# Gorilla-Lab-SCUT/frustum-convnet

Measured on AMD Instinct MI355X. Metric: frustums/sec (train fwd+bwd) KITTI-car B=32 N=1024, higher is better.
Workload: dtype f32 (fp32 operands split into two 16-bit parts, 3 MFMAs per product, fp32 accumulate); 1 GPU; cfgs/det_sample.yaml KITTI-car, batch=32/GPU, Npoint=1024, L=(280,140,70,35), train fwd+bwd+Adam; global_batch=32, parallelism=dp1

## Files before the change

frustum_convnet_amd/csrc/fcn_tuning.h:

```cpp
#pragma once

#ifndef FCN_EXP
#define FCN_EXP 0
#endif
#define MM_ENC_W ((FCN_EXP & 1) ? MM_F32 : MM)
#define MM_ENC_A ((FCN_EXP & 2) ? MM_F32 : MM)

#ifndef FCN_X
#define FCN_X 0
#endif

#ifndef FCN_XB
#define FCN_XB 0
#endif

#ifndef FCN_XF
#define FCN_XF 0
#endif
#ifndef FCN_XG
#define FCN_XG 0
#endif

#ifdef FCN_TUNING_PNF
#ifdef FCN_PROBE
// ... 18 lines not shown
    unsigned int n = 0;
    if (hipMemcpyFromSymbol(&n, HIP_SYMBOL(g_pnf_probe_n), sizeof(n)) != hipSuccess) return -1;
    if ((int)n > max_records) n = max_records;
    if (n > PNF_MAX) n = PNF_MAX;
    if (n && hipMemcpyFromSymbol(host_out, HIP_SYMBOL(g_pnf_probe), (size_t)n * 8 * sizeof(unsigned long long)) != hipSuccess) return -1;
    if (reset) { unsigned int z = 0; hipMemcpyToSymbol(HIP_SYMBOL(g_pnf_probe_n), &z, sizeof(z)); }
    return (int)n;
}
#else
#define PNF_DECL
#define PNF_ADD(i)
#define PNF_FLUSH(tag)
#endif
#endif

#ifdef FCN_TUNING_PNP
#ifdef FCN_PROBE
#define PNP_MAX 32768
__device__ unsigned long long g_pn_probe[PNP_MAX * 8];
__device__ unsigned int g_pn_probe_n;
#define PNP_DECL unsigned long long pa_[6] = {0, 0, 0, 0, 0, 0}; unsigned long long pt_ = clock64(), pt0_ = pt_
#define PNP_ADD(i) do { const unsigned long long n_ = clock64(); pa_[i] += n_ - pt_; pt_ = n_; } while (0)
#define PNP_FLUSH(tag)                                                                                   \
    do {                                                                                                 \
        if (threadIdx.x == 0) {                                                                          \
            const unsigned int s_ = atomicAdd(&g_pn_probe_n, 1u);                                        \
            if (s_ < PNP_MAX) {                                                                          \
                g_pn_probe[s_ * 8] = (unsigned long long)(tag);                                          \
                g_pn_probe[s_ * 8 + 1] = clock64() - pt0_;                                               \
                for (int q_ = 0; q_ < 6; ++q_) g_pn_probe[s_ * 8 + 2 + q_] = pa_[q_];                    \
            }                                                                                            \
        }                                                                                                \
    } while (0)
extern "C" int fcn_pn_probe_read(unsigned long long *host_out, int max_records, int reset)
{
    unsigned int n = 0;
    if (hipMemcpyFromSymbol(&n, HIP_SYMBOL(g_pn_probe_n), sizeof(n)) != hipSuccess) return -1;
    if ((int)n > max_records) n = max_records;
    if (n > PNP_MAX) n = PNP_MAX;
    if (n && hipMemcpyFromSymbol(host_out, HIP_SYMBOL(g_pn_probe), (size_t)n * 8 * sizeof(unsigned long long)) != hipSuccess) return -1;
    if (reset) { unsigned int z = 0; hipMemcpyToSymbol(HIP_SYMBOL(g_pn_probe_n), &z, sizeof(z)); }
    return (int)n;
}
#else
#define PNP_DECL
#define PNP_ADD(i)
#define PNP_FLUSH(tag)
#endif
#endif

#ifdef FCN_TUNING_FCN
#ifdef FCN_PROBE
#define FCN_PROBE_MAX 65536
__device__ unsigned long long g_fcn_probe[FCN_PROBE_MAX * 8];
__device__ unsigned int g_fcn_probe_n;
#define PROBE_DECL unsigned long long pb_[8]; int pbn_ = 0
#define PROBE_STAMP() do { if (pbn_ < 7) pb_[pbn_++] = wall_clock64(); } while (0)
#define PROBE_FLUSH(tag)                                                                                 \
    do {                                                                                                 \
        if (threadIdx.x == 0) {                                                                          \
            const unsigned int s_ = atomicAdd(&g_fcn_probe_n, 1u);                                       \
            if (s_ < FCN_PROBE_MAX) {                                                                    \
                g_fcn_probe[s_ * 8] = (unsigned long long)(tag);                                         \
                for (int q_ = 0; q_ < 7; ++q_) g_fcn_probe[s_ * 8 + 1 + q_] = q_ < pbn_ ? pb_[q_] : 0ull; \
            }                                                                                            \
        }                                                                                                \
    } while (0)
extern "C" int fcn_probe_read(unsigned long long *host_out, int max_records, int reset)
{
    unsigned int n = 0;
    if (hipMemcpyFromSymbol(&n, HIP_SYMBOL(g_fcn_probe_n), sizeof(n)) != hipSuccess) return -1;
    if ((int)n > max_records) n = max_records;
    if (n > FCN_PROBE_MAX) n = FCN_PROBE_MAX;
    if (n && hipMemcpyFromSymbol(host_out, HIP_SYMBOL(g_fcn_probe), (size_t)n * 8 * sizeof(unsigned long long)) != hipSuccess) return -1;
    if (reset) { unsigned int z = 0; hipMemcpyToSymbol(HIP_SYMBOL(g_fcn_probe_n), &z, sizeof(z)); }
    return (int)n;
}
#else
#define PROBE_DECL
#define PROBE_STAMP()
#define PROBE_FLUSH(tag)
#endif
#if defined(FCN_PROBE) && FCN_PROBE >= 3
#define BPROBE_DECL unsigned long long pb_[8]; int pbn_ = 0
#define BPROBE_STAMP() do { if (pbn_ < 7) pb_[pbn_++] = wall_clock64(); } while (0)
#define BPROBE_FLUSH(tag) PROBE_FLUSH(tag)
#else
#define BPROBE_DECL
#define BPROBE_STAMP()
#define BPROBE_FLUSH(tag)
#endif
#endif

#ifndef FCN_POOL_FUSED
#define FCN_POOL_FUSED 1
#endif
```

frustum_convnet_amd/csrc/gemm_tile.h:

```cpp
#pragma once
#include "fcn_common.h"
#include "fcn_tuning.h"

typedef float v4f __attribute__((ext_vector_type(4)));
typedef int v4i __attribute__((ext_vector_type(4)));
typedef const v4f __attribute__((address_space(1))) *gv4fp;
typedef const v4i __attribute__((address_space(1))) *gv4ip;
__device__ __forceinline__ v4f ldg4(const float *p) { return *(gv4fp)p; }
__device__ __forceinline__ v4i ldg4i(const int *p) { return *(gv4ip)p; }
__device__ __forceinline__ void sts4(float *p, v4f v) { *(v4f *)p = v; }
__device__ __forceinline__ v4f zero4() { v4f z = {0.f, 0.f, 0.f, 0.f}; return z; }


#define GT 256

static inline bool fcn_pn_key_pool(const fcn_pn_desc *d, const fcn_pn_ws *ws, int C3)
{
    return FCN_POOL_FUSED && d->nlc && ws->pkey && ws->ewin && C3 % 2 == 0 && C3 <= 2 * GT && (2 * GT) % C3 == 0;
}
#define KC 32

#define MM_F32 0
#define MM_F16X3 1
#define MM_BF16X3 2
// ... 236 lines not shown
    } else {
#pragma unroll
        for (int q = 0; q < 4; ++q) {
            float h, l;
            enc2<MM>(x[2 * q], x[2 * q + 1], h, l);
            hi[q] = __builtin_bit_cast(uint32_t, h);
            lo[q] = __builtin_bit_cast(uint32_t, l);
        }
    }
}

typedef float v2f_kb __attribute__((ext_vector_type(2)));
template <int MM, int LDR>
__device__ __forceinline__ void kb_store4(u32x4 *img, int r, int kq, float x0, float x1, float x2, float x3)
{
    const int kb = kq >> 1, half = kq & 1;
    if constexpr (MM == MM_F32) {
        const v4f v = {x0, x1, x2, x3};
        *(v4f *)(img + (half * 4 + kb) * LDR + r) = v;
    } else {
        float h0, l0, h1, l1;
        enc2<MM>(x0, x1, h0, l0);
        enc2<MM>(x2, x3, h1, l1);
        const v2f_kb h = {h0, h1}, l = {l0, l1};
        *(v2f_kb *)((float *)(img + kb * LDR + r) + 2 * half) = h;
        if constexpr (!mm_x1<MM>) *(v2f_kb *)((float *)(img + (4 + kb) * LDR + r) + 2 * half) = l;
    }
}

typedef const u32x4 __attribute__((address_space(1))) *gu4p;
__device__ __forceinline__ u32x4 ldgu4(const u32x4 *p) { return *(gu4p)p; }

template <int MM, int MT, int NT, int LDRA, int LDRB>
__device__ __forceinline__ void mma_chunk_kb(const u32x4 *A, const u32x4 *B, int arow0, int bcol0, f32x16 (&acc)[MT][NT])
{
    const int lane = threadIdx.x & 63;
    const int l31 = lane & 31, lh = lane >> 5;
    if constexpr (MM == MM_F32) {
        const float *Af = (const float *)A, *Bf = (const float *)B;
#pragma unroll
        for (int kk = 0; kk < KC; kk += 2) {
            const int k = kk + lh, kb = k >> 3, j = k & 7;
            float a[MT], b[NT];
#pragma unroll
            for (int i = 0; i < MT; ++i) a[i] = Af[(((j >> 2) * 4 + kb) * LDRA + arow0 + i * 32 + l31) * 4 + (j & 3)];
#pragma unroll
            for (int jn = 0; jn < NT; ++jn) b[jn] = Bf[(((j >> 2) * 4 + kb) * LDRB + bcol0 + jn * 32 + l31) * 4 + (j & 3)];
#pragma unroll
            for (int i = 0; i < MT; ++i)
#pragma unroll
                for (int jn = 0; jn < NT; ++jn)
                    acc[i][jn] = __builtin_amdgcn_mfma_f32_32x32x2f32(a[i], b[jn], acc[i][jn], 0, 0, 0);
        }
    } else {
        constexpr bool X3 = !mm_x1<MM>;
        const u32x4 *ap = A + lh * LDRA + arow0 + l31;
        const u32x4 *bp = B + lh * LDRB + bcol0 + l31;
#pragma unroll
        for (int ks = 0; ks < 2; ++ks) {
            u32x4 ah[MT], al[MT], bh[NT], bl[NT];
#pragma unroll
            for (int i = 0; i < MT; ++i) {
                ah[i] = ap[2 * ks * LDRA + i * 32];
                if constexpr (X3) al[i] = ap[(4 + 2 * ks) * LDRA + i * 32];
            }
#pragma unroll
            for (int j = 0; j < NT; ++j) {
                bh[j] = bp[2 * ks * LDRB + j * 32];
                if constexpr (X3) bl[j] = bp[(4 + 2 * ks) * LDRB + j * 32];
            }
            if constexpr (X3) {
#pragma unroll
                for (int i = 0; i < MT; ++i)
#pragma unroll
                    for (int j = 0; j < NT; ++j) acc[i][j] = mfma16<MM>(ah[i], bl[j], acc[i][j]);
#pragma unroll
                for (int i = 0; i < MT; ++i)
#pragma unroll
                    for (int j = 0; j < NT; ++j) acc[i][j] = mfma16<MM>(al[i], bh[j], acc[i][j]);
            }
#pragma unroll
            for (int i = 0; i < MT; ++i)
#pragma unroll
                for (int j = 0; j < NT; ++j) acc[i][j] = mfma16<MM>(ah[i], bh[j], acc[i][j]);
        }
    }
}

#define EP_LD 32
#define EP_FLOATS (32 * EP_LD)
__device__ __forceinline__ void ep_put(float *patch, const f32x16 &acc, int l31, int lh)
{
#pragma unroll
    for (int reg = 0; reg < 16; ++reg) patch[acc_row_c(reg, lh) * EP_LD + l31] = acc[reg];
}
__device__ __forceinline__ v4f ep_get(const float *patch, int lane, int q)
{
    const int idx = lane + 64 * q;
    return *(const v4f *)(patch + (idx >> 3) * EP_LD + 4 * (idx & 7));
}

#define FCN_MM_OF(prec, fwd)                                                                     \
    ((prec) == FCN_PREC_F32 ? MM_F32 : ((prec) == FCN_PREC_BF16 ? MM_BF16S : ((prec) == FCN_PREC_BF16_OPS ? MM_BF16X1 : ((fwd) ? MM_F16X3 : MM_BF16X3))))
#define FCN_MM_SWITCH(mm_, CALL)                                     \
    switch (mm_) {                                                   \
        case MM_F32: { constexpr int MM = MM_F32; CALL; } break;     \
        case MM_F16X3: { constexpr int MM = MM_F16X3; CALL; } break; \
        case MM_BF16X3: { constexpr int MM = MM_BF16X3; CALL; } break; \
        case MM_BF16X1: { constexpr int MM = MM_BF16X1; CALL; } break; \
        default: { constexpr int MM = MM_BF16S; CALL; } break;       \
    }

__device__ __forceinline__ int fcn_xcd_tile(int id, int n)
{
    const int per = (n + 7) >> 3;
    const int t = (id & 7) * per + (id >> 3);
    return (t < n && (id >> 3) < per) ? t : -1;
}

// ... 6 lines not shown
```

frustum_convnet_amd/csrc/pointnet_bwd.hip:

```cpp
#define FCN_TUNING_PNP
#include "gemm_tile.h"

#define LDT 129
#define MAXC 512
#define WG_ROWS 128
#define WG_TMAX 256
#define PWB 16
#ifndef FCN_WIDE_TILES
#define FCN_WIDE_TILES 0
#endif
#ifndef FCN_DG_WIDE
#define FCN_DG_WIDE 1
#endif
#ifndef FCN_WG_PITCH_PAD
#define FCN_WG_PITCH_PAD 0
#endif
#ifndef FCN_WG3_OCC
#define FCN_WG3_OCC 3
#endif
#ifndef FCN_WG2_OCC
#define FCN_WG2_OCC 2
#endif
#ifndef FCN_DG2_OCC
#define FCN_DG2_OCC 3
#endif

extern "C" int fcn_pn_wgrad_rows(void) { return WG_ROWS; }
extern "C" int fcn_stat_replicas(void) { return FCN_STAT_REP; }


template <int S16>
__global__ __launch_bounds__(GT) void poolbwd_kernel(
    const float *__restrict__ dfeat, const int32_t *__restrict__ amax, const float *__restrict__ y3,
    const float *__restrict__ bn3, float *__restrict__ gmax, double *__restrict__ bstat, int rep_stride,
// ... 46 lines not shown
    __syncthreads();
    if (tid < 64) {
        double a = 0.0, g = 0.0;
        for (int w = 0; w < 4; ++w) {
            a += (double)red[(w * 64 + tid) * 2];
            g += (double)red[(w * 64 + tid) * 2 + 1];
        }
        double *br = bstat + (int64_t)((blockIdx.x + blockIdx.z) % FCN_STAT_REP) * rep_stride;
        atomic_add_f64(&br[c0 + tid], a);
        atomic_add_f64(&br[C3 + c0 + tid], g);
    }
}

struct DgradArgs {
    const float4 *ent;
    const int32_t *woff;
    const int32_t *tiles;
    const int32_t *ewin;
    const float *ycur;
    const int32_t *amax;
    const float *gmax;
    const float *dzcur;
    FcnBnBwd cb;
    const u32x4 *Wenc;
    float *dybuf;
    const float *yprev;
    const float *bn_prev;
    const float *W1;
    float *dzprev;
    double *bstat_prev;
    int L, cap, CRED, CPREV, tps;
};

template <int MT, int NT, int WN>
struct DgradLds {
    static constexpr int TM = 64 * MT, TN = 32 * NT * WN;
    static constexpr int U4 = KbTile<TM>::U4 + KbTile<TN>::U4;
    static constexpr int BYTES = U4 * 16 + 5 * MAXC * 4 + TM * 16;
};

template <int MM, int LAYER, int MT, int NT, int WN, int DZ3 = 0>
__device__ __forceinline__ void dgrad_body(const DgradArgs &a, const int bid, unsigned char *smem_)
{
    static_assert(!DZ3 || LAYER == 3, "DZ3 is a form of the layer-3 data gradient");
    constexpr bool MAPS = LAYER == 3 && !DZ3;
    constexpr int NTHR = 128 * WN;
    constexpr int TM = 64 * MT;
    constexpr int TN = 32 * NT * WN;
    constexpr int LDRA = KbTile<TM>::LDR, LDRB = KbTile<TN>::LDR;
    constexpr int NA4 = TM * 8 / NTHR;
    constexpr int NB = TN * 8 / NTHR;
    constexpr int SUB = 128 / TM;
    constexpr int LDSU4 = KbTile<TM>::U4 + KbTile<TN>::U4;
    u32x4 *lds4 = (u32x4 *)smem_;
    float *coefS = (float *)(smem_ + LDSU4 * 16);
    float4 *uS = (float4 *)(smem_ + LDSU4 * 16 + 5 * MAXC * 4);
    u32x4 *Ab = lds4, *Bb = lds4 + KbTile<TM>::U4;

    const int tid = threadIdx.x, lane = tid & 63, wave = tid >> 6;
    const int l31 = lane & 31, lh = lane >> 5;
    const int wm = wave / WN, wn = wave % WN;
    const int ny = a.CPREV / TN;
    if (bid == 0 && a.cb.dgamma) {
        for (int c = tid; c < a.CRED; c += NTHR) {
            a.cb.dgamma[c] = (float)fcn_rep_sum(a.cb.bstat + a.CRED + c, a.cb.rep_stride);
            a.cb.dbeta[c] = (float)fcn_rep_sum(a.cb.bstat + c, a.cb.rep_stride);
        }
    }
    const int xt = fcn_xcd_tile(bid, SUB * a.tiles[0] * ny);
    if (xt < 0) return;
    const int bxi = xt / ny, byi = xt % ny;
    const int lt = bxi / SUB, sub = bxi % SUB;
    const int code = a.tiles[4 + lt];
    const int b = code / a.tps, t = code % a.tps;
    const int nent = a.woff[(int64_t)b * (a.L + 1) + a.L];
    const int row0 = t * 128 + sub * TM;
    const int nvalid = min(TM, nent - row0);
    if (nvalid <= 0) return;
    const int64_t grow0 = (int64_t)b * a.cap + row0;
    const int k0 = byi * TN;
    const int CRED = a.CRED, CPREV = a.CPREV;

    PNP_DECL;
    for (int c = tid; c < CRED; c += NTHR) {
        float cf[5];
        fcn_bnbwd_coef(a.cb, CRED, c, cf, false);
#pragma unroll
        for (int q = 0; q < 5; ++q) coefS[q * CRED + c] = cf[q];
    }
    if (tid < TM) uS[tid] = (tid < nvalid) ? a.ent[grow0 + tid] : make_float4(0.f, 0.f, 0.f, 0.f);
    unsigned arowB[NA4];
    unsigned wbaseB[NA4];
#pragma unroll
    for (int i = 0; i < NA4; ++i) {
        const int f = tid + NTHR * i;
        const int rc = min(f >> 3, nvalid - 1);
        arowB[i] = (unsigned)(rc * CRED + 4 * (f & 7)) * St<MM>::bytes;
        wbaseB[i] = 0;
        if constexpr (MAPS) wbaseB[i] = (unsigned)(a.ewin[grow0 + rc] * CRED + 4 * (f & 7)) * 4u;
    }
    const int64_t tile0 = grow0 * CRED;
    const int64_t map0 = (int64_t)b * a.L * CRED;
    __syncthreads();

    f32x16 acc[MT][NT];
    acc_zero<MT, NT>(acc);
    v4f ry[NA4], rz[NA4];
    v4i rm[NA4];
    u32x4 rw[NB];
    const int nchunk = CRED / KC;
    unsigned woffB[NB];
#pragma unroll
    for (int i = 0; i < NB; ++i) woffB[i] = (unsigned)((tid % TN) + (tid / TN + i * (NTHR / TN)) * CPREV) * 16u;
    const u32x4 *wsrc = a.Wenc + k0;

#define DGRAD_LOAD(cc)                                                                                                \
    {                                                                                                                 \
        const int nq_ = (cc) * KC;                                                                                    \
        if (!((FCN_XB & 1) && (cc) > 0))                                                                              \
        {                                                                                                             \
            const float *yb_ = st_ptr<MM>(a.ycur, tile0 + nq_);                                                       \
            const int *mb_ = MAPS ? a.amax + map0 + nq_ : nullptr;                                                    \
            const float *gb_ = MAPS ? a.gmax + map0 + nq_ : st_ptr<MM>(a.dzcur, tile0 + nq_);                         \
            _Pragma("unroll") for (int i = 0; i < NA4; ++i) {                                                         \
                ry[i] = lds4b<MM>(yb_, arowB[i]);                                                                     \
                if constexpr (MAPS) {                                                                                 \
                    rm[i] = *(gv4ip)((const char *)mb_ + fcn_opaque_v32(wbaseB[i]));                                  \
                    rz[i] = *(gv4fp)((const char *)gb_ + fcn_opaque_v32(wbaseB[i]));                                  \
                } else {                                                                                              \
                    rz[i] = lds4b<MM>(gb_, arowB[i]);                                                                 \
                }                                                                                                     \
            }                                                                                                         \
        }                                                                                                             \
        if (!((FCN_XB & 2) && (cc) > 0))                                                                              \
        {                                                                                                             \
            const char *wb_ = (const char *)(wsrc + (int64_t)(cc) * 8 * CPREV);                                       \
            _Pragma("unroll") for (int i = 0; i < NB; ++i) rw[i] = *(gu4p)(wb_ + fcn_opaque_v32(woffB[i]));           \
        }                                                                                                             \
    }

    PNP_ADD(0);
    DGRAD_LOAD(0);
    for (int c = 0; c < nchunk; ++c) {
        PNP_ADD(1);
        if ((FCN_XB & 4) && c > 0) goto staged;
#pragma unroll
        for (int i = 0; i < NA4; ++i) {
            const int f = tid + NTHR * i;
            const int r = f >> 3, kq = f & 7;
            const bool ok = r < nvalid;
            const float w = uS[r].w;
            const int rloc = row0 + r;
            const float yv[4] = {ry[i].x, ry[i].y, ry[i].z, ry[i].w};
            const float zv[4] = {rz[i].x, rz[i].y, rz[i].z, rz[i].w};
            int mv[4] = {0, 0, 0, 0};
            if constexpr (MAPS) { mv[0] = rm[i].x; mv[1] = rm[i].y; mv[2] = rm[i].z; mv[3] = rm[i].w; }
            const int nb = c * KC + 4 * kq;
            float cfv[4][4];
#pragma unroll
            for (int q = 0; q < 4; ++q) {
                const v4f c4 = *(const v4f *)(coefS + q * CRED + nb);
                cfv[q][0] = c4.x; cfv[q][1] = c4.y; cfv[q][2] = c4.z; cfv[q][3] = c4.w;
            }
            float dv[4];
#pragma unroll
            for (int j = 0; j < 4; ++j) {
                float dz = zv[j];
                if constexpr (MAPS) dz = (mv[j] == rloc) ? zv[j] : 0.f;
                dv[j] = fcn_bn_dy(cfv[0][j], cfv[1][j], cfv[2][j], cfv[3][j], dz, yv[j], w);
            }
            kb_store4<MM_ENC_A, LDRA>(Ab, r, kq, dv[0], dv[1], dv[2], dv[3]);
            if constexpr (LAYER == 3) {
                if (ok && byi == 0 && a.dybuf && !(FCN_XB & 128)) {
                    const v4f d0 = {dv[0], dv[1], dv[2], dv[3]};
                    sts4e<MM>(a.dybuf, (grow0 + r) * CRED + nb, d0);
                }
            }
        }
#pragma unroll
        for (int i = 0; i < NB; ++i) {
            const int f = tid + NTHR * i;
            Bb[(f / TN) * LDRB + (f % TN)] = rw[i];
        }
    staged:
        PNP_ADD(2);
        __syncthreads();
        PNP_ADD(3);
        if (c + 1 < nchunk) DGRAD_LOAD(c + 1);
        PNP_ADD(1);
        if (!(FCN_XB & 8)) mma_chunk_kb<MM, MT, NT, LDRA, LDRB>(Ab, Bb, wm * 32 * MT, wn * 32 * NT, acc);
        PNP_ADD(4);
        __syncthreads();
        PNP_ADD(3);
    }
#undef DGRAD_LOAD

    PNP_ADD(3);
    if (FCN_XB & 16) { if (acc[0][0][0] == 123.456f) a.bstat_prev[0] = 0.0; return; }
    constexpr int NS = (LAYER == 3) ? 2 : 4;
    float st[NT][NS];
#pragma unroll
    for (int nt = 0; nt < NT; ++nt) {
        const int col = k0 + wn * 32 * NT + nt * 32 + l31;
        const float ps = a.bn_prev[col], pt = a.bn_prev[CPREV + col];
#pragma unroll
        for (int q = 0; q < NS; ++q) st[nt][q] = 0.f;
        if constexpr (LAYER == 3) {
            const float pm = a.bn_prev[2 * CPREV + col], pr = a.bn_prev[3 * CPREV + col];
            float yv[MT][16];
#pragma unroll
            for (int mt = 0; mt < MT; ++mt)
#pragma unroll
                for (int reg = 0; reg < 16; ++reg) {
                    const int row = min(wm * 32 * MT + mt * 32 + acc_row(reg, lh), nvalid - 1);
                    yv[mt][reg] = lds1e<MM>(a.yprev, (grow0 + row) * CPREV + col);
                }
#pragma unroll
            for (int mt = 0; mt < MT; ++mt)
#pragma unroll
                for (int reg = 0; reg < 16; ++reg) {
                    const int row = wm * 32 * MT + mt * 32 + acc_row(reg, lh);
                    if (row < nvalid) {
                        const float y = yv[mt][reg];
                        const float dz = st_round<MM>((fmaf(ps, y, pt) > 0.f) ? acc[mt][nt][reg] : 0.f);
                        if (!(FCN_XB & 32)) sts1e<MM>(a.dzprev, (grow0 + row) * CPREV + col, dz);
                        st[nt][0] += dz;
                        st[nt][1] = fmaf(dz, (y - pm) * pr, st[nt][1]);
                    }
                }
        } else {
            const float al[3] = {ps * a.W1[3 * col], ps * a.W1[3 * col + 1], ps * a.W1[3 * col + 2]};
#pragma unroll
            for (int mt = 0; mt < MT; ++mt)
#pragma unroll
                for (int reg = 0; reg < 16; ++reg) {
                    const int row = wm * 32 * MT + mt * 32 + acc_row(reg, lh);
                    if (row < nvalid) {
                        const float4 u = uS[row];
                        const float dz = (l1_pre(al, pt, u.x, u.y, u.z) > 0.f) ? acc[mt][nt][reg] : 0.f;
                        st[nt][0] += dz;
                        st[nt][1] = fmaf(dz, u.x, st[nt][1]);
                        st[nt][2] = fmaf(dz, u.y, st[nt][2]);
                        st[nt][3] = fmaf(dz, u.z, st[nt][3]);
                    }
                }
        }
#pragma unroll
        for (int q = 0; q < NS; ++q) st[nt][q] += __shfl_xor(st[nt][q], 32, 64);
    }
    PNP_ADD(5);
    float *red = (float *)lds4;
    if (wm == 1 && lh == 0) {
#pragma unroll
        for (int nt = 0; nt < NT; ++nt)
#pragma unroll
            for (int q = 0; q < NS; ++q) red[(((wn * NT + nt) * 32 + l31) * NS) + q] = st[nt][q];
    }
    __syncthreads();
    if (wm == 0 && lh == 0) {
#pragma unroll
        for (int nt = 0; nt < NT; ++nt) {
            const int col = k0 + wn * 32 * NT + nt * 32 + l31;
#pragma unroll
            for (int q = 0; q < NS; ++q) {
                const double v = (double)st[nt][q] + (double)red[(((wn * NT + nt) * 32 + l31) * NS) + q];
                double *br = a.bstat_prev + (int64_t)fcn_rep_id() * a.cb.rep_stride;
                if (!(FCN_XB & 64)) atomic_add_f64(&br[q * CPREV + col], v);
                else if (v == 123.456) br[0] = v;
            }
        }
    }
    PNP_FLUSH(((unsigned long long)LAYER << 48) | ((unsigned long long)CRED << 32) | ((unsigned long long)CPREV << 16) |
              (unsigned long long)nvalid);
}

template <int MM, int LAYER, int MT, int NT, int WN, int DZ3 = 0>
__global__ __launch_bounds__(128 * WN) __attribute__((amdgpu_waves_per_eu(MT * NT <= 2 ? (LAYER == 2 ? FCN_DG2_OCC : 3) : 2, 4)))
void dgrad_kernel(DgradArgs a)
{
    __shared__ __attribute__((aligned(16))) unsigned char smem[DgradLds<MT, NT, WN>::BYTES];
    dgrad_body<MM, LAYER, MT, NT, WN, DZ3>(a, (int)blockIdx.x, smem);
}

struct WgradArgs {
    const float4 *ent;
    const int32_t *woff;
    const int32_t *tiles;
    const float *dy;
    const float *dz;
    const float *ycur;
    FcnBnBwd cb;
    const int32_t *ewin;
    const int32_t *amax;
    const float *gmax;
    const float *yprev;
    const float *bn_prev;
    const float *W1;
    float *partial;
    int L, cap, COUT, CIN, tps;
};

template <int MM>
__device__ __forceinline__ float4 ld4f(const float *base, int64_t e)
{
    const v4f v = lds4e<MM>(base, e);
    return make_float4(v.x, v.y, v.z, v.w);
}

template <int MM>
__device__ __forceinline__ float4 ld4fb(const float *sbase, unsigned boff)
{
    const v4f v = lds4b<MM>(sbase, boff);
    return make_float4(v.x, v.y, v.z, v.w);
}
// ... 222 lines not shown
#pragma unroll
            for (int reg = 0; reg < 16; ++reg) {
                const int n = n0 + wm * 32 * MT + mt * 32 + acc_row(reg, lh);
                const int k = k0 + wn * 32 * NT + nt * 32 + l31;
                out[(int64_t)n * CIN + k] = acc[mt][nt][reg];
            }
    PNP_FLUSH(((unsigned long long)(10 + LAYER) << 48) | ((unsigned long long)COUT << 32) | ((unsigned long long)CIN << 16) |
              (unsigned long long)64);
}

template <int MM, int LAYER, int MT, int NT, int RC = 0>
__global__ __launch_bounds__(GT) __attribute__((amdgpu_waves_per_eu((LAYER == 3 && !RC) ? FCN_WG3_OCC : FCN_WG2_OCC, 4))) void wgrad_kernel(WgradArgs a)
{
    __shared__ __attribute__((aligned(16))) unsigned char smem[WgradLds<MT, NT, RC>::BYTES];
    wgrad_body<MM, LAYER, MT, NT, RC>(a, (int)blockIdx.x, (int)blockIdx.y, (int)blockIdx.z, (int)gridDim.x, smem);
}

struct PnMidArgs {
    DgradArgs g2;
    WgradArgs w3, w2;
    int n_g2, n_w3;
    int ns3, oy3, ns2, oy2;
};
template <int A, int B>
struct CMax { static constexpr int V = A > B ? A : B; };

template <int MM, int DNT, int W3M, int W3N, int W2M, int W2N>
__global__ __launch_bounds__(GT) __attribute__((amdgpu_waves_per_eu(2, 4))) void pn_mid_kernel(PnMidArgs m)
{
    constexpr int LB = CMax<CMax<DgradLds<1, DNT, 2>::BYTES, WgradLds<W3M, W3N, 0>::BYTES>::V, WgradLds<W2M, W2N, 0>::BYTES>::V;
    __shared__ __attribute__((aligned(16))) unsigned char smem[LB];
    const int bid = (int)blockIdx.x;
    if (bid < m.n_g2) {
        dgrad_body<MM, 2, 1, DNT, 2>(m.g2, bid, smem);
    } else if (bid < m.n_g2 + m.n_w3) {
        const int i = bid - m.n_g2, bx = i % m.ns3, r = i / m.ns3;
        wgrad_body<MM, 3, W3M, W3N, 0>(m.w3, bx, r % m.oy3, r / m.oy3, m.ns3, smem);
    } else {
        const int i = bid - m.n_g2 - m.n_w3, bx = i % m.ns2, r = i / m.ns2;
        wgrad_body<MM, 2, W2M, W2N, 0>(m.w2, bx, r % m.oy2, r / m.oy2, m.ns2, smem);
    }
}

#define WR_T 256
struct ReduceJob {
    const float *partial;
    const int32_t *tiles;
    float *out;
    int64_t nelem;
    int nsplit, gr, nblk;
};
__device__ __forceinline__ void wgrad_reduce_body(const ReduceJob &j, const int rid, float *sh)
{
    const int gr = j.gr, per = WR_T / gr;
    const int x = threadIdx.x % per, y = threadIdx.x / per;
    const int64_t i = ((int64_t)rid * per + x) * 4;
    const int ntile = j.tiles[0];
    const int tpb = (ntile + j.nsplit - 1) / j.nsplit;
    const int nsp = tpb > 0 ? (ntile + tpb - 1) / tpb : 0;
    const float *p = j.partial + i;
    const int64_t nelem = j.nelem;
    v4f s0 = zero4(), s1 = zero4(), s2 = zero4(), s3 = zero4();
    int sp = y;
    for (; sp + 3 * gr < nsp; sp += 4 * gr) {
        s0 += ldg4(p + (int64_t)sp * nelem);
        s1 += ldg4(p + (int64_t)(sp + gr) * nelem);
        s2 += ldg4(p + (int64_t)(sp + 2 * gr) * nelem);
// ... 38 lines not shown
    const double mean = a.bn1[2 * C + c], rstd = a.bn1[3 * C + c];
    const double db = q0;
    const double dg = rstd * (w[0] * qu[0] + w[1] * qu[1] + w[2] * qu[2] - mean * q0);
    const double iM = 1.0 / a.M;
    const double mu[3] = {mom[1] * iM, mom[2] * iM, mom[3] * iM};
    const double m2[3][3] = {{mom[4] * iM, mom[5] * iM, mom[6] * iM},
                             {mom[5] * iM, mom[7] * iM, mom[8] * iM},
                             {mom[6] * iM, mom[8] * iM, mom[9] * iM}};
    const double kk = (double)a.gamma[c] * rstd;
    for (int j = 0; j < 3; ++j) {
        const double wm2 = w[0] * m2[0][j] + w[1] * m2[1][j] + w[2] * m2[2][j];
        const double v = a.frozen ? kk * qu[j] : kk * (qu[j] - db * mu[j] - dg * rstd * (wm2 - mean * mu[j]));
        a.dW1[3 * c + j] = (float)v;
    }
    a.dgamma[c] = (float)dg;
    a.dbeta[c] = (float)db;
}
__global__ void l1_finalize_kernel(L1Args a) { l1_finalize_body(a, (int)(blockIdx.x * blockDim.x + threadIdx.x)); }

struct PnTailArgs {
    ReduceJob r[2];
    L1Args l1;
    int has_l1;
};
__global__ __launch_bounds__(WR_T) void pn_tail_kernel(PnTailArgs t)
{
    __shared__ __attribute__((aligned(16))) float sh[WR_T * 4];
    const int bid = (int)blockIdx.x;
    if (bid < t.r[0].nblk) wgrad_reduce_body(t.r[0], bid, sh);
    else if (bid < t.r[0].nblk + t.r[1].nblk) wgrad_reduce_body(t.r[1], bid - t.r[0].nblk, sh);
    else if (t.has_l1) l1_finalize_body(t.l1, (bid - t.r[0].nblk - t.r[1].nblk) * WR_T + (int)threadIdx.x);
}

template <int LAYER, int DZ3 = 0>
static int launch_dgrad(const DgradArgs &a, int B, int precision, hipStream_t st)
{
    if (a.CRED % 64 || a.CPREV % 64 || a.CRED > MAXC) return FCN_E_BADARG;
    if ((int64_t)B * a.cap * (a.CRED > a.CPREV ? a.CRED : a.CPREV) >= (int64_t)1 << 31) return FCN_E_LIMIT;
    const unsigned nt = (unsigned)(B * a.tps);
#if FCN_DG_WIDE
    if (a.CPREV % 256 == 0) {
        FCN_MM_SWITCH(FCN_MM_OF(precision, false),
                      hipLaunchKernelGGL((dgrad_kernel<MM, LAYER, 1, 2, 4, DZ3>), dim3((2 * nt * (a.CPREV / 256) + 7) / 8 * 8), dim3(512), 0, st, a));
        FCN_CHECK_LAUNCH();
        return 0;
    }
#endif
    if (a.CPREV % 128 == 0) {
        FCN_MM_SWITCH(FCN_MM_OF(precision, false),
                      hipLaunchKernelGGL((dgrad_kernel<MM, LAYER, 1, 2, 2, DZ3>), dim3((2 * nt * (a.CPREV / 128) + 7) / 8 * 8), dim3(256), 0, st, a));
    } else {
        FCN_MM_SWITCH(FCN_MM_OF(precision, false),
                      hipLaunchKernelGGL((dgrad_kernel<MM, LAYER, 1, 1, 2, DZ3>), dim3((2 * nt * (a.CPREV / 64) + 7) / 8 * 8), dim3(256), 0, st, a));
    }
    FCN_CHECK_LAUNCH();
    return 0;
}

template <int MM, int LAYER, int RC = 0>
static void launch_wgrad_mm(const WgradArgs &a, dim3 grid, bool m2, bool n2, hipStream_t st)
{
    if (m2 && n2) hipLaunchKernelGGL((wgrad_kernel<MM, LAYER, 2, 2, RC>), grid, dim3(GT), 0, st, a);
    else if (m2) hipLaunchKernelGGL((wgrad_kernel<MM, LAYER, 2, 1, RC>), grid, dim3(GT), 0, st, a);
    else if (n2) hipLaunchKernelGGL((wgrad_kernel<MM, LAYER, 1, 2, RC>), grid, dim3(GT), 0, st, a);
    else hipLaunchKernelGGL((wgrad_kernel<MM, LAYER, 1, 1, RC>), grid, dim3(GT), 0, st, a);
}

struct WgradPlan {
    int nsplit, oy, oz;
    bool m2, n2;
};

template <int LAYER>
static int plan_wgrad(const WgradArgs &a, int B, int nsplit_cap, WgradPlan &P)
{
    P.m2 = (a.COUT % 128 == 0); P.n2 = (a.CIN % 128 == 0);
    P.oy = a.COUT / (P.m2 ? 128 : 64); P.oz = a.CIN / (P.n2 ? 128 : 64);
#ifndef FCN_WG_SLOTS
#define FCN_WG_SLOTS 256
#endif
    const int slots = (LAYER == 2 && P.m2 && P.n2) ? (FCN_WG_SLOTS * 2) / 3 : FCN_WG_SLOTS;
    if ((int64_t)B * a.cap * (a.COUT > a.CIN ? a.COUT : a.CIN) >= (int64_t)1 << 31) return FCN_E_LIMIT;
    if ((int64_t)B * a.cap >= (int64_t)1 << 24) return FCN_E_LIMIT;
    int nsplit = slots / (P.oy * P.oz);
    if (nsplit < (B * a.tps + WG_TMAX - 1) / WG_TMAX) nsplit = (B * a.tps + WG_TMAX - 1) / WG_TMAX;
    if (nsplit < 1) nsplit = 1;
// ... 316 lines not shown
```

Measured before the change: 29150 frustums/s.

## Pipeline PointNet dgrad chunks with double-buffered LDS and persistent tile loop

The PointNet backward data-gradient kernel now double-buffers the A tile in LDS and splits each K-chunk MMA into two halves. Staging and global loads for the next chunk (weights in two halves) are interleaved between those halves to hide memory latency behind MFMA work. The kernel also becomes persistent: the grid is capped at CU count times occupancy and each workgroup loops over tiles, computing BN coefficients once per workgroup. This costs more LDS per block and a dedicated reduction buffer, and changes the stat replica index to come from the tile id.

After: 28460 frustums/s. 2.4% lower.

```diff
diff --git a/frustum_convnet_amd/csrc/fcn_tuning.h b/frustum_convnet_amd/csrc/fcn_tuning.h
--- a/frustum_convnet_amd/csrc/fcn_tuning.h
+++ b/frustum_convnet_amd/csrc/fcn_tuning.h
@@ -74,6 +74,7 @@
             }                                                                                            \
         }                                                                                                \
     } while (0)
+#define PNP_RESET do { for (int q_ = 0; q_ < 6; ++q_) pa_[q_] = 0; pt_ = pt0_ = clock64(); } while (0)
 extern "C" int fcn_pn_probe_read(unsigned long long *host_out, int max_records, int reset)
 {
     unsigned int n = 0;
@@ -88,6 +89,7 @@
 #define PNP_DECL
 #define PNP_ADD(i)
 #define PNP_FLUSH(tag)
+#define PNP_RESET
 #endif
 #endif
 
@@ -134,6 +136,13 @@
 #endif
 #endif
 
+#ifndef FCN_DG_PIPE
+#define FCN_DG_PIPE 1
+#endif
+#ifndef FCN_DG_BHALF
+#define FCN_DG_BHALF 1
+#endif
+
 #ifndef FCN_POOL_FUSED
 #define FCN_POOL_FUSED 1
 #endif
diff --git a/frustum_convnet_amd/csrc/gemm_tile.h b/frustum_convnet_amd/csrc/gemm_tile.h
--- a/frustum_convnet_amd/csrc/gemm_tile.h
+++ b/frustum_convnet_amd/csrc/gemm_tile.h
@@ -292,14 +292,14 @@
 __device__ __forceinline__ u32x4 ldgu4(const u32x4 *p) { return *(gu4p)p; }
 
 template <int MM, int MT, int NT, int LDRA, int LDRB>
-__device__ __forceinline__ void mma_chunk_kb(const u32x4 *A, const u32x4 *B, int arow0, int bcol0, f32x16 (&acc)[MT][NT])
+__device__ __forceinline__ void mma_half_kb(const u32x4 *A, const u32x4 *B, int arow0, int bcol0, f32x16 (&acc)[MT][NT], const int ks)
 {
     const int lane = threadIdx.x & 63;
     const int l31 = lane & 31, lh = lane >> 5;
     if constexpr (MM == MM_F32) {
         const float *Af = (const float *)A, *Bf = (const float *)B;
 #pragma unroll
-        for (int kk = 0; kk < KC; kk += 2) {
+        for (int kk = ks * (KC / 2); kk < (ks + 1) * (KC / 2); kk += 2) {
             const int k = kk + lh, kb = k >> 3, j = k & 7;
             float a[MT], b[NT];
 #pragma unroll
@@ -316,8 +316,7 @@
         constexpr bool X3 = !mm_x1<MM>;
         const u32x4 *ap = A + lh * LDRA + arow0 + l31;
         const u32x4 *bp = B + lh * LDRB + bcol0 + l31;
-#pragma unroll
-        for (int ks = 0; ks < 2; ++ks) {
+        {
             u32x4 ah[MT], al[MT], bh[NT], bl[NT];
 #pragma unroll
             for (int i = 0; i < MT; ++i) {
@@ -345,6 +344,13 @@
                 for (int j = 0; j < NT; ++j) acc[i][j] = mfma16<MM>(ah[i], bh[j], acc[i][j]);
         }
     }
+}
+
+template <int MM, int MT, int NT, int LDRA, int LDRB>
+__device__ __forceinline__ void mma_chunk_kb(const u32x4 *A, const u32x4 *B, int arow0, int bcol0, f32x16 (&acc)[MT][NT])
+{
+    mma_half_kb<MM, MT, NT, LDRA, LDRB>(A, B, arow0, bcol0, acc, 0);
+    mma_half_kb<MM, MT, NT, LDRA, LDRB>(A, B, arow0, bcol0, acc, 1);
 }
 
 #define EP_LD 32
diff --git a/frustum_convnet_amd/csrc/pointnet_bwd.hip b/frustum_convnet_amd/csrc/pointnet_bwd.hip
--- a/frustum_convnet_amd/csrc/pointnet_bwd.hip
+++ b/frustum_convnet_amd/csrc/pointnet_bwd.hip
@@ -1,5 +1,6 @@
 #define FCN_TUNING_PNP
 #include "gemm_tile.h"
+#include <type_traits>
 
 #define LDT 129
 #define MAXC 512
@@ -112,15 +113,16 @@
     int L, cap, CRED, CPREV, tps;
 };
 
-template <int MT, int NT, int WN>
+template <int MT, int NT, int WN, int PIPE = FCN_DG_PIPE>
 struct DgradLds {
     static constexpr int TM = 64 * MT, TN = 32 * NT * WN;
-    static constexpr int U4 = KbTile<TM>::U4 + KbTile<TN>::U4;
-    static constexpr int BYTES = U4 * 16 + 5 * MAXC * 4 + TM * 16;
+    static constexpr int U4 = (PIPE ? 2 : 1) * KbTile<TM>::U4 + KbTile<TN>::U4;
+    static constexpr int RED = WN * NT * 32 * 4;
+    static constexpr int BYTES = U4 * 16 + 5 * MAXC * 4 + TM * 16 + RED * 4;
 };
 
-template <int MM, int LAYER, int MT, int NT, int WN, int DZ3 = 0>
-__device__ __forceinline__ void dgrad_body(const DgradArgs &a, const int bid, unsigned char *smem_)
+template <int MM, int LAYER, int MT, int NT, int WN, int DZ3 = 0, int PIPE = FCN_DG_PIPE>
+__device__ __forceinline__ void dgrad_body(const DgradArgs &a, const int bid, const int nwg, unsigned char *smem_)
 {
     static_assert(!DZ3 || LAYER == 3, "DZ3 is a form of the layer-3 data gradient");
     constexpr bool MAPS = LAYER == 3 && !DZ3;
@@ -131,24 +133,53 @@
     constexpr int NA4 = TM * 8 / NTHR;
     constexpr int NB = TN * 8 / NTHR;
     constexpr int SUB = 128 / TM;
-    constexpr int LDSU4 = KbTile<TM>::U4 + KbTile<TN>::U4;
+    constexpr int AU4 = KbTile<TM>::U4;
+    constexpr int LDSU4 = DgradLds<MT, NT, WN, PIPE>::U4;
+    static_assert(NTHR % TN == 0 && (NTHR / TN == 2 || NTHR / TN == 4), "weight image items of a thread: see b_half");
     u32x4 *lds4 = (u32x4 *)smem_;
     float *coefS = (float *)(smem_ + LDSU4 * 16);
     float4 *uS = (float4 *)(smem_ + LDSU4 * 16 + 5 * MAXC * 4);
-    u32x4 *Ab = lds4, *Bb = lds4 + KbTile<TM>::U4;
-
-    const int tid = threadIdx.x, lane = tid & 63, wave = tid >> 6;
+    float *red = (float *)(smem_ + LDSU4 * 16 + 5 * MAXC * 4 + TM * 16);
+    u32x4 *Ab = lds4, *Bb = lds4 + (PIPE ? 2 : 1) * AU4;
+
+    const int ny = a.CPREV / TN;
+    const int CRED = a.CRED, CPREV = a.CPREV;
+    if (bid == 0 && a.cb.dgamma) {
+        for (int c = threadIdx.x; c < CRED; c += NTHR) {
+            a.cb.dgamma[c] = (float)fcn_rep_sum(a.cb.bstat + CRED + c, a.cb.rep_stride);
+            a.cb.dbeta[c] = (float)fcn_rep_sum(a.cb.bstat + c, a.cb.rep_stride);
+        }
+    }
+    const int ntile = SUB * a.tiles[0] * ny;
+    const int id_end = ((ntile + 7) >> 3) << 3;
+    if (bid >= id_end) return;
+
+    PNP_DECL;
+    for (int c = threadIdx.x; c < CRED; c += NTHR) {
+        float cf[5];
+        fcn_bnbwd_coef(a.cb, CRED, c, cf, false);
+#pragma unroll
+        for (int q = 0; q < 5; ++q) coefS[q * CRED + c] = cf[q];
+    }
+    const int nchunk = CRED / KC;
+
+    for (int id = bid; id < id_end; id += nwg) {
+    int tid = threadIdx.x;
+#ifndef FCN_HOST_EMU
+    asm volatile("" : "+v"(tid));
+#endif
+    const int lane = tid & 63, wave = tid >> 6;
     const int l31 = lane & 31, lh = lane >> 5;
     const int wm = wave / WN, wn = wave % WN;
-    const int ny = a.CPREV / TN;
-    if (bid == 0 && a.cb.dgamma) {
-        for (int c = tid; c < a.CRED; c += NTHR) {
-            a.cb.dgamma[c] = (float)fcn_rep_sum(a.cb.bstat + a.CRED + c, a.cb.rep_stride);
-            a.cb.dbeta[c] = (float)fcn_rep_sum(a.cb.bstat + c, a.cb.rep_stride);
-        }
-    }
-    const int xt = fcn_xcd_tile(bid, SUB * a.tiles[0] * ny);
-    if (xt < 0) return;
+    unsigned woffB[NB];
+#pragma unroll
+    for (int i = 0; i < NB; ++i) woffB[i] = (unsigned)((tid % TN) + (tid / TN + i * (NTHR / TN)) * CPREV) * 16u;
+    auto b_half = [&](int i) __attribute__((always_inline)) {
+        if constexpr (NTHR / TN == 2) return i & 1;
+        else return (tid / TN >> 1) & 1;
+    };
+    const int xt = fcn_xcd_tile(id, ntile);
+    if (xt < 0) continue;
     const int bxi = xt / ny, byi = xt % ny;
     const int lt = bxi / SUB, sub = bxi % SUB;
     const int code = a.tiles[4 + lt];
@@ -156,18 +187,10 @@
     const int nent = a.woff[(int64_t)b * (a.L + 1) + a.L];
     const int row0 = t * 128 + sub * TM;
     const int nvalid = min(TM, nent - row0);
-    if (nvalid <= 0) return;
+    if (nvalid <= 0) continue;
     const int64_t grow0 = (int64_t)b * a.cap + row0;
     const int k0 = byi * TN;
-    const int CRED = a.CRED, CPREV = a.CPREV;
-
-    PNP_DECL;
-    for (int c = tid; c < CRED; c += NTHR) {
-        float cf[5];
-        fcn_bnbwd_coef(a.cb, CRED, c, cf, false);
-#pragma unroll
-        for (int q = 0; q < 5; ++q) coefS[q * CRED + c] = cf[q];
-    }
+
     if (tid < TM) uS[tid] = (tid < nvalid) ? a.ent[grow0 + tid] : make_float4(0.f, 0.f, 0.f, 0.f);
     unsigned arowB[NA4];
     unsigned wbaseB[NA4];
@@ -181,49 +204,39 @@
     }
     const int64_t tile0 = grow0 * CRED;
     const int64_t map0 = (int64_t)b * a.L * CRED;
-    __syncthreads();
 
     f32x16 acc[MT][NT];
     acc_zero<MT, NT>(acc);
     v4f ry[NA4], rz[NA4];
     v4i rm[NA4];
     u32x4 rw[NB];
-    const int nchunk = CRED / KC;
-    unsigned woffB[NB];
-#pragma unroll
-    for (int i = 0; i < NB; ++i) woffB[i] = (unsigned)((tid % TN) + (tid / TN + i * (NTHR / TN)) * CPREV) * 16u;
     const u32x4 *wsrc = a.Wenc + k0;
 
-#define DGRAD_LOAD(cc)                                                                                                \
-    {                                                                                                                 \
-        const int nq_ = (cc) * KC;                                                                                    \
-        if (!((FCN_XB & 1) && (cc) > 0))                                                                              \
-        {                                                                                                             \
-            const float *yb_ = st_ptr<MM>(a.ycur, tile0 + nq_);                                                       \
-            const int *mb_ = MAPS ? a.amax + map0 + nq_ : nullptr;                                                    \
-            const float *gb_ = MAPS ? a.gmax + map0 + nq_ : st_ptr<MM>(a.dzcur, tile0 + nq_);                         \
-            _Pragma("unroll") for (int i = 0; i < NA4; ++i) {                                                         \
-                ry[i] = lds4b<MM>(yb_, arowB[i]);                                                                     \
-                if constexpr (MAPS) {                                                                                 \
-                    rm[i] = *(gv4ip)((const char *)mb_ + fcn_opaque_v32(wbaseB[i]));                                  \
-                    rz[i] = *(gv4fp)((const char *)gb_ + fcn_opaque_v32(wbaseB[i]));                                  \
-                } else {                                                                                              \
-                    rz[i] = lds4b<MM>(gb_, arowB[i]);                                                                 \
-                }                                                                                                     \
-            }                                                                                                         \
-        }                                                                                                             \
-        if (!((FCN_XB & 2) && (cc) > 0))                                                                              \
-        {                                                                                                             \
-            const char *wb_ = (const char *)(wsrc + (int64_t)(cc) * 8 * CPREV);                                       \
-            _Pragma("unroll") for (int i = 0; i < NB; ++i) rw[i] = *(gu4p)(wb_ + fcn_opaque_v32(woffB[i]));           \
-        }                                                                                                             \
-    }
-
-    PNP_ADD(0);
-    DGRAD_LOAD(0);
-    for (int c = 0; c < nchunk; ++c) {
-        PNP_ADD(1);
-        if ((FCN_XB & 4) && c > 0) goto staged;
+    auto load_a = [&](int cc) __attribute__((always_inline)) {
+        const int nq_ = cc * KC;
+        if ((FCN_XB & 1) && cc > 0) return;
+        const float *yb_ = st_ptr<MM>(a.ycur, tile0 + nq_);
+        const int *mb_ = MAPS ? a.amax + map0 + nq_ : nullptr;
+        const float *gb_ = MAPS ? a.gmax + map0 + nq_ : st_ptr<MM>(a.dzcur, tile0 + nq_);
+#pragma unroll
+        for (int i = 0; i < NA4; ++i) {
+            ry[i] = lds4b<MM>(yb_, arowB[i]);
+            if constexpr (MAPS) {
+                rm[i] = *(gv4ip)((const char *)mb_ + fcn_opaque_v32(wbaseB[i]));
+                rz[i] = *(gv4fp)((const char *)gb_ + fcn_opaque_v32(wbaseB[i]));
+            } else {
+                rz[i] = lds4b<MM>(gb_, arowB[i]);
+            }
+        }
+    };
+    auto load_w = [&](int cc, int h) __attribute__((always_inline)) {
+        if ((FCN_XB & 2) && cc > 0) return;
+        const char *wb_ = (const char *)(wsrc + (int64_t)cc * 8 * CPREV);
+#pragma unroll
+        for (int i = 0; i < NB; ++i)
+            if (h == 2 || b_half(i) == h) rw[i] = *(gu4p)(wb_ + fcn_opaque_v32(woffB[i]));
+    };
+    auto stage_a = [&](int cc, u32x4 *img) __attribute__((always_inline)) {
 #pragma unroll
         for (int i = 0; i < NA4; ++i) {
             const int f = tid + NTHR * i;
@@ -235,7 +248,7 @@
             const float zv[4] = {rz[i].x, rz[i].y, rz[i].z, rz[i].w};
             int mv[4] = {0, 0, 0, 0};
             if constexpr (MAPS) { mv[0] = rm[i].x; mv[1] = rm[i].y; mv[2] = rm[i].z; mv[3] = rm[i].w; }
-            const int nb = c * KC + 4 * kq;
+            const int nb = cc * KC + 4 * kq;
             float cfv[4][4];
 #pragma unroll
             for (int q = 0; q < 4; ++q) {
@@ -249,7 +262,7 @@
                 if constexpr (MAPS) dz = (mv[j] == rloc) ? zv[j] : 0.f;
                 dv[j] = fcn_bn_dy(cfv[0][j], cfv[1][j], cfv[2][j], cfv[3][j], dz, yv[j], w);
             }
-            kb_store4<MM_ENC_A, LDRA>(Ab, r, kq, dv[0], dv[1], dv[2], dv[3]);
+            kb_store4<MM_ENC_A, LDRA>(img, r, kq, dv[0], dv[1], dv[2], dv[3]);
             if constexpr (LAYER == 3) {
                 if (ok && byi == 0 && a.dybuf && !(FCN_XB & 128)) {
                     const v4f d0 = {dv[0], dv[1], dv[2], dv[3]};
@@ -257,25 +270,82 @@
                 }
             }
         }
+    };
+    auto stage_w = [&](int h) __attribute__((always_inline)) {
 #pragma unroll
         for (int i = 0; i < NB; ++i) {
             const int f = tid + NTHR * i;
-            Bb[(f / TN) * LDRB + (f % TN)] = rw[i];
-        }
-    staged:
+            if (h == 2 || b_half(i) == h) Bb[(f / TN) * LDRB + (f % TN)] = rw[i];
+        }
+    };
+
+    PNP_ADD(0);
+    load_a(0);
+    load_w(0, 2);
+    PNP_ADD(1);
+    __syncthreads();
+    PNP_ADD(3);
+    if constexpr (PIPE) {
+        stage_a(0, Ab);
+        stage_w(2);
         PNP_ADD(2);
+        if (nchunk > 1) { load_w(1, FCN_DG_BHALF ? 0 : 2); load_a(1); if (FCN_DG_BHALF) load_w(1, 1); }
+        PNP_ADD(1);
         __syncthreads();
         PNP_ADD(3);
-        if (c + 1 < nchunk) DGRAD_LOAD(c + 1);
-        PNP_ADD(1);
-        if (!(FCN_XB & 8)) mma_chunk_kb<MM, MT, NT, LDRA, LDRB>(Ab, Bb, wm * 32 * MT, wn * 32 * NT, acc);
-        PNP_ADD(4);
-        __syncthreads();
-        PNP_ADD(3);
-    }
-#undef DGRAD_LOAD
-
-    PNP_ADD(3);
+        auto chunk = [&](const int c, auto NXT, auto NXT2) __attribute__((always_inline)) {
+            constexpr bool nxt = decltype(NXT)::value, nxt2 = decltype(NXT2)::value;
+            const u32x4 *Ac = Ab + (c & 1) * AU4;
+            u32x4 *An = Ab + ((c + 1) & 1) * AU4;
+            if (!(FCN_XB & 8)) mma_half_kb<MM, MT, NT, LDRA, LDRB>(Ac, Bb, wm * 32 * MT, wn * 32 * NT, acc, 0);
+            PNP_ADD(4);
+            if constexpr (FCN_DG_BHALF && nxt) {
+                __syncthreads();
+                PNP_ADD(3);
+                stage_w(0);
+                PNP_ADD(2);
+                if constexpr (nxt2) load_w(c + 2, 0);
+                PNP_ADD(1);
+            }
+            if constexpr (nxt) {
+                stage_a(c + 1, An);
+                PNP_ADD(2);
+                if constexpr (nxt2) load_a(c + 2);
+                PNP_ADD(1);
+            }
+            if (!(FCN_XB & 8)) mma_half_kb<MM, MT, NT, LDRA, LDRB>(Ac, Bb, wm * 32 * MT, wn * 32 * NT, acc, 1);
+            PNP_ADD(4);
+            if constexpr (nxt) {
+                __syncthreads();
+                PNP_ADD(3);
+                stage_w(FCN_DG_BHALF ? 1 : 2);
+                PNP_ADD(2);
+                if constexpr (nxt2) load_w(c + 2, FCN_DG_BHALF ? 1 : 2);
+                PNP_ADD(1);
+                if constexpr (!FCN_DG_BHALF) { __syncthreads(); PNP_ADD(3); }
+            }
+        };
+        typedef std::integral_constant<bool, true> Yes;
+        typedef std::integral_constant<bool, false> No;
+        for (int c = 0; c + 2 < nchunk; ++c) chunk(c, Yes(), Yes());
+        chunk(nchunk - 2, Yes(), No());
+        chunk(nchunk - 1, No(), No());
+    } else {
+        for (int c = 0; c < nchunk; ++c) {
+            if (c > 0) __syncthreads();
+            PNP_ADD(3);
+            stage_a(c, Ab);
+            stage_w(2);
+            PNP_ADD(2);
+            __syncthreads();
+            PNP_ADD(3);
+            if (c + 1 < nchunk) { load_a(c + 1); load_w(c + 1, 2); }
+            PNP_ADD(1);
+            if (!(FCN_XB & 8)) mma_chunk_kb<MM, MT, NT, LDRA, LDRB>(Ab, Bb, wm * 32 * MT, wn * 32 * NT, acc);
+            PNP_ADD(4);
+        }
+    }
+
     if (FCN_XB & 16) { if (acc[0][0][0] == 123.456f) a.bstat_prev[0] = 0.0; return; }
     constexpr int NS = (LAYER == 3) ? 2 : 4;
     float st[NT][NS];
@@ -329,7 +399,6 @@
         for (int q = 0; q < NS; ++q) st[nt][q] += __shfl_xor(st[nt][q], 32, 64);
     }
     PNP_ADD(5);
-    float *red = (float *)lds4;
     if (wm == 1 && lh == 0) {
 #pragma unroll
         for (int nt = 0; nt < NT; ++nt)
@@ -344,7 +413,7 @@
 #pragma unroll
             for (int q = 0; q < NS; ++q) {
                 const double v = (double)st[nt][q] + (double)red[(((wn * NT + nt) * 32 + l31) * NS) + q];
-                double *br = a.bstat_prev + (int64_t)fcn_rep_id() * a.cb.rep_stride;
+                double *br = a.bstat_prev + (int64_t)(id % FCN_STAT_REP) * a.cb.rep_stride;
                 if (!(FCN_XB & 64)) atomic_add_f64(&br[q * CPREV + col], v);
                 else if (v == 123.456) br[0] = v;
             }
@@ -352,14 +421,16 @@
     }
     PNP_FLUSH(((unsigned long long)LAYER << 48) | ((unsigned long long)CRED << 32) | ((unsigned long long)CPREV << 16) |
               (unsigned long long)nvalid);
+    PNP_RESET;
+    }
 }
 
 template <int MM, int LAYER, int MT, int NT, int WN, int DZ3 = 0>
-__global__ __launch_bounds__(128 * WN) __attribute__((amdgpu_waves_per_eu(MT * NT <= 2 ? (LAYER == 2 ? FCN_DG2_OCC : 3) : 2, 4)))
+__global__ __launch_bounds__(128 * WN) __attribute__((amdgpu_waves_per_eu(WN == 4 ? 4 : (MT * NT <= 2 ? (LAYER == 2 ? FCN_DG2_OCC : 3) : 2), 4)))
 void dgrad_kernel(DgradArgs a)
 {
     __shared__ __attribute__((aligned(16))) unsigned char smem[DgradLds<MT, NT, WN>::BYTES];
-    dgrad_body<MM, LAYER, MT, NT, WN, DZ3>(a, (int)blockIdx.x, smem);
+    dgrad_body<MM, LAYER, MT, NT, WN, DZ3>(a, (int)blockIdx.x, (int)gridDim.x, smem);
 }
 
 struct WgradArgs {
@@ -648,7 +719,7 @@
     __shared__ __attribute__((aligned(16))) unsigned char smem[LB];
     const int bid = (int)blockIdx.x;
     if (bid < m.n_g2) {
-        dgrad_body<MM, 2, 1, DNT, 2>(m.g2, bid, smem);
+        dgrad_body<MM, 2, 1, DNT, 2>(m.g2, bid, m.n_g2, smem);
     } else if (bid < m.n_g2 + m.n_w3) {
         const int i = bid - m.n_g2, bx = i % m.ns3, r = i / m.ns3;
         wgrad_body<MM, 3, W3M, W3N, 0>(m.w3, bx, r % m.oy3, r / m.oy3, m.ns3, smem);
@@ -753,26 +824,50 @@
     else if (t.has_l1) l1_finalize_body(t.l1, (bid - t.r[0].nblk - t.r[1].nblk) * WR_T + (int)threadIdx.x);
 }
 
+template <int MM, int LAYER, int MT, int NT, int WN, int DZ3>
+static void launch_dgrad_mm(const DgradArgs &a, unsigned ntile_max, hipStream_t st)
+{
+    constexpr int NTHR = 128 * WN;
+    unsigned slots = ntile_max;
+#ifndef FCN_HOST_EMU
+    static int cached = 0;
+    if (!cached) {
+        int dev = 0, ncu = 0, occ = 0;
+        if (hipGetDevice(&dev) == hipSuccess && hipDeviceGetAttribute(&ncu, hipDeviceAttributeMultiprocessorCount, dev) == hipSuccess &&
+            hipOccupancyMaxActiveBlocksPerMultiprocessor(&occ, dgrad_kernel<MM, LAYER, MT, NT, WN, DZ3>, NTHR, 0) == hipSuccess && ncu > 0 && occ > 0)
+            cached = ncu * occ;
+        else
+            cached = -1;
+        (void)hipGetLastError();
+    }
+    if (cached > 0 && (unsigned)cached < slots) slots = (unsigned)cached;
+#endif
+    unsigned grid = (slots + 7) / 8 * 8;
+    if (const char *e = getenv("FCN_DG_GRID")) {
+        const long v = atol(e);
+        if (v >= 1) grid = (unsigned)(v < (long)ntile_max ? v : (long)ntile_max);
+    }
+    hipLaunchKernelGGL((dgrad_kernel<MM, LAYER, MT, NT, WN, DZ3>), dim3(grid), dim3(NTHR), 0, st, a);
+}
+
 template <int LAYER, int DZ3 = 0>
 static int launch_dgrad(const DgradArgs &a, int B, int precision, hipStream_t st)
 {
     if (a.CRED % 64 || a.CPREV % 64 || a.CRED > MAXC) return FCN_E_BADARG;
     if ((int64_t)B * a.cap * (a.CRED > a.CPREV ? a.CRED : a.CPREV) >= (int64_t)1 << 31) return FCN_E_LIMIT;
+    if ((int64_t)a.L * a.CRED * 4 >= (int64_t)1 << 32 || (int64_t)B * a.tps * (a.CPREV / 64) >= (int64_t)1 << 28) return FCN_E_LIMIT;
     const unsigned nt = (unsigned)(B * a.tps);
 #if FCN_DG_WIDE
     if (a.CPREV % 256 == 0) {
-        FCN_MM_SWITCH(FCN_MM_OF(precision, false),
-                      hipLaunchKernelGGL((dgrad_kernel<MM, LAYER, 1, 2, 4, DZ3>), dim3((2 * nt * (a.CPREV / 256) + 7) / 8 * 8), dim3(512), 0, st, a));
+        FCN_MM_SWITCH(FCN_MM_OF(precision, false), (launch_dgrad_mm<MM, LAYER, 1, 2, 4, DZ3>(a, (2 * nt * (a.CPREV / 256) + 7) / 8 * 8, st)));
         FCN_CHECK_LAUNCH();
         return 0;
     }
 #endif
     if (a.CPREV % 128 == 0) {
-        FCN_MM_SWITCH(FCN_MM_OF(precision, false),
-                      hipLaunchKernelGGL((dgrad_kernel<MM, LAYER, 1, 2, 2, DZ3>), dim3((2 * nt * (a.CPREV / 128) + 7) / 8 * 8), dim3(256), 0, st, a));
+        FCN_MM_SWITCH(FCN_MM_OF(precision, false), (launch_dgrad_mm<MM, LAYER, 1, 2, 2, DZ3>(a, (2 * nt * (a.CPREV / 128) + 7) / 8 * 8, st)));
     } else {
-        FCN_MM_SWITCH(FCN_MM_OF(precision, false),
-                      hipLaunchKernelGGL((dgrad_kernel<MM, LAYER, 1, 1, 2, DZ3>), dim3((2 * nt * (a.CPREV / 64) + 7) / 8 * 8), dim3(256), 0, st, a));
+        FCN_MM_SWITCH(FCN_MM_OF(precision, false), (launch_dgrad_mm<MM, LAYER, 1, 1, 2, DZ3>(a, (2 * nt * (a.CPREV / 64) + 7) / 8 * 8, st)));
     }
     FCN_CHECK_LAUNCH();
     return 0;
```
